# azrael417/mlperf-deepcam

Hardware: AMD Instinct MI355X
Metric: samples/sec (768x1152x16) train step (higher is better)
Workload: dtype bf16; 1 GPU; DeepLabV3+/Xception train step (fwd + weighted CE + bwd + LAMB), 768x1152x16, local_batch=8, bf16 activations / fp32 master weights, random-init seed 333; local_batch=8, global_batch=8, parallelism=dp1, optimizer=LAMB, hip_graph=False, launch_list_replay=False

## Files before the change

mlperf-deepcam_amd/csrc/common.h:

```cpp
#pragma once
#include <hip/hip_runtime.h>
#include <stdint.h>

#include <mutex>

#include "../../include/deepcam_hip.h"

namespace dc {

typedef __bf16 bf16;
typedef __attribute__((ext_vector_type(8))) __bf16 bf16x8;
typedef __attribute__((ext_vector_type(4))) __bf16 bf16x4;
typedef __attribute__((ext_vector_type(4))) short short4v;
typedef __attribute__((ext_vector_type(4))) float f32x4;
typedef __attribute__((ext_vector_type(2))) float f32x2;

struct alignas(16) vec16 {
  uint32_t w[4];
};

template <typename T>
struct Elem;
template <>
struct Elem<float> {
  static constexpr int kPerVec = 4;
  static constexpr int kDtype = DC_F32;
  __device__ static inline float load(const float* p) { return *p; }
  __device__ static inline void store(float* p, float v) { *p = v; }
};
template <>
struct Elem<bf16> {
  static constexpr int kPerVec = 8;
  static constexpr int kDtype = DC_BF16;
  __device__ static inline float load(const bf16* p) { return (float)*p; }
  __device__ static inline void store(bf16* p, float v) { *p = (bf16)v; }
};

__device__ inline void unpack(const vec16& v, float (&f)[4], float) {
#pragma unroll
  for (int i = 0; i < 4; ++i) f[i] = __uint_as_float(v.w[i]);
}
__device__ inline void unpack(const vec16& v, float (&f)[8], bf16) {
#pragma unroll
  for (int i = 0; i < 4; ++i) {
    f[2 * i] = __uint_as_float(v.w[i] << 16);
    f[2 * i + 1] = __uint_as_float(v.w[i] & 0xffff0000u);
  }
}
__device__ inline uint32_t pack2_bf16(float lo, float hi) {
  typedef __attribute__((ext_vector_type(2))) __bf16 bf16x2;
  bf16x2 r;
  r[0] = (bf16)lo;
  r[1] = (bf16)hi;
  return __builtin_bit_cast(uint32_t, r);
}
__device__ inline void pack(vec16& v, const float (&f)[4], float) {
#pragma unroll
  for (int i = 0; i < 4; ++i) v.w[i] = __float_as_uint(f[i]);
}
__device__ inline void pack(vec16& v, const float (&f)[8], bf16) {
#pragma unroll
  for (int i = 0; i < 4; ++i) v.w[i] = pack2_bf16(f[2 * i], f[2 * i + 1]);
}

__device__ inline vec16 zero16() {
  vec16 z;
  z.w[0] = z.w[1] = z.w[2] = z.w[3] = 0u;
  return z;
}
__device__ inline vec16 ldg16(const void* p) { return *reinterpret_cast<const vec16*>(p); }
__device__ inline void stg16(void* p, const vec16& v) { *reinterpret_cast<vec16*>(p) = v; }

__device__ inline float wave_sum(float v) {
#pragma unroll
  for (int o = 32; o > 0; o >>= 1) v += __shfl_xor(v, o, 64);
  return v;
}
__device__ inline double wave_sum(double v) {
#pragma unroll
  for (int o = 32; o > 0; o >>= 1) v += __shfl_xor(v, o, 64);
  return v;
}

inline int cdiv(long a, long b) { return (int)((a + b - 1) / b); }

struct Options {
  int igemm256 = 1;
  int igemm256p = 1;
  int igemm256p_wgs = 0;
  int igemm256p_min = 257;
  int igemm256_splitk = 1;
  int pw384 = 1;
  int pw224 = 1;
  int pw192 = 1;
  int thin_tile = 1;
  int wgrad384 = 1;
  int wgrad384_slots = 192;
  int wgrad384_min_stages = 96;
  int head_fused = 1;
  int head_dgrad_fused = 1;
  int head_wgrad_fused = 1;
  int dw_tile = 1;
  int dw_wgrad_tpb = 0;
  int dw_pipe = 1;
  int bn_apply_rows = 1;
};
extern Options g_options;

const void* zero_page(hipError_t* err);

}

#define DC_ONCE(...)                               \
  do {                                             \
    static std::once_flag once_flag__;             \
    std::call_once(once_flag__, [&] { __VA_ARGS__; }); \
  } while (0)

namespace dc {
extern thread_local bool g_launch_log_on;
void launch_log_note(const char* name);
}

#define DC_LAUNCHED(name)                                  \
  do {                                                     \
    hipError_t e__ = hipGetLastError();                    \
    if (e__ != hipSuccess) return dc_set_error(e__, __FILE__, __LINE__); \
    if (dc::g_launch_log_on) dc::launch_log_note(name);    \
  } while (0)
#define DC_CHECK_LAUNCH() DC_LAUNCHED("aux")

extern "C" int dc_set_error(int code, const char* file, int line);
extern "C" int dc_fail(const char* msg, const char* file, int line);
extern "C" int dc_check_view(const void* ptr, int ld, int c, int dtype, const char* what);
#define DC_REQUIRE(cond, msg)                                  \
  do {                                                         \
    if (!(cond)) return dc_fail(msg, __FILE__, __LINE__);      \
  } while (0)
```

mlperf-deepcam_amd/csrc/igemm.h:

```cpp
#pragma once
#include "conv_geom.h"

namespace dc {

constexpr int WLD_ALIGN = 64;
__host__ __device__ inline int weight_ld(int c) {
  const int a = c < 64 ? 32 : WLD_ALIGN;
  return (c + a - 1) / a * a;
}


struct BnBwdEpi {
  const void* y;
  int ldy;
  const float* mean;
  const float* invstd;
  const float* mscale;
  const float* mshift;
  int relu;
};

struct IgemmParams {
  const void* x;
  const void* w;
  void* y;
  const float* bias;
  float* slab;
  GatherGeom g;
  int N, ldx, ldy;
  int ldw;
  const void* w_kn = nullptr;
  int ldw_kn = 0;
  int M;
  int m_beg = 0;
  int mtiles;
  int accumulate = 0;
  const void* zero_page = nullptr;
  static constexpr int MAXGROUP = 4;
  BnBwdEpi bst{};
  int ngroup = 0;
  int gdil[MAXGROUP];
  const void* gw[MAXGROUP - 1];
  void* gy[MAXGROUP - 1];
  float* gslab[MAXGROUP - 1];
  int ksplit = 0;
  float* kslab = nullptr;
  int zfill = 0;
};

int launch_igemm256(const IgemmParams& p, hipStream_t st);
bool igemm256p_eligible(const IgemmParams& p);
int launch_igemm256p(const IgemmParams& p, int workgroups, hipStream_t st);
inline long igemm256_tiles(const IgemmParams& p) {
  return (long)((p.g.Cout + 255) / 256) * ((p.M - p.m_beg + 255) / 256) * p.g.os * p.g.os * (p.ngroup > 1 ? p.ngroup : 1);
}
int igemm256_splitk_plan(const IgemmParams& p, size_t* slab_bytes);
int launch_igemm256_splitk(const IgemmParams& p, int splits, void* ws, hipStream_t st);

bool pw384_eligible(const IgemmParams& p);
int launch_pw384(const IgemmParams& p, int npb, hipStream_t st);
inline long pw384_tiles(const IgemmParams& p, int npb) { return (long)((p.g.Cout + 383) / 384) * ((p.M + 32 * npb - 1) / (32 * npb)); }

bool pw224_eligible(const IgemmParams& p);
int launch_pw224(const IgemmParams& p, int tn, hipStream_t st);
inline long pw224_tiles(const IgemmParams& p, int tn = 384) { return (long)((p.g.Cout + tn - 1) / tn) * ((p.M + 223) / 224); }

long pw192_tiles(const IgemmParams& p);
int launch_pw192(const IgemmParams& p, hipStream_t st);

bool thin_fwd_eligible(const GatherGeom& g, int dtype, int bias, int accumulate, int out32);
int launch_thin_fwd(const GatherGeom& g, int N, const void* in, int ldin, const void* w, int ldw, void* out, int ldout, float* slab,
                    int slab_rows, hipStream_t st);

}
```

mlperf-deepcam_amd/csrc/igemm.hip:

```cpp
#include <stdio.h>
#include <string.h>

#include <type_traits>

#include "conv_geom.h"
#include "igemm.h"
#include "mfma_tile.h"

namespace dc {

constexpr int BM = 128, BN = 128;
constexpr int ROWB = 64, NSTAGE = 3;

template <typename T>
struct Mma;
template <>
struct Mma<bf16> {
  __device__ static inline void run(const vec16& a, const vec16& b, f32x4& c) {
    c = __builtin_amdgcn_mfma_f32_16x16x32_bf16(__builtin_bit_cast(bf16x8, a), __builtin_bit_cast(bf16x8, b), c, 0, 0, 0);
  }
};
template <>
struct Mma<float> {
  __device__ static inline void run(const vec16& a, const vec16& b, f32x4& c) {
// ... 665 lines not shown
    int lo = 0, hi = nentries;
    while (hi - lo > 1) {
      const int mid = (lo + hi) >> 1;
      if (prefix[mid] <= gt) lo = mid; else hi = mid;
    }
    const PackEntry e = table[lo];
    const int tile = gt - prefix[lo];
    if (e.kind == 2) {
      float* out = reinterpret_cast<float*>(e.wf);
      const int c = tile * 256 + threadIdx.x;
      if (c < e.cout) {
#pragma unroll
        for (int t = 0; t < 9; ++t) out[(size_t)t * e.cout + c] = e.master[(size_t)c * 9 + t];
      }
      continue;
    }
    if (e.taps == 1) {
      if constexpr (sizeof(T) == 2) {
        if (((e.cin | e.cout) & 7) == 0) pack_pointwise_tile_bf16(e, tile, lds);
        else pack_dense_tile<T, 1>(e, tile, lds);
      } else {
        pack_dense_tile<T, 1>(e, tile, lds);
      }
    } else {
      pack_dense_tile<T, 9>(e, tile, lds);
    }
  }
}

}

using namespace dc;

constexpr int PACK_BLOCKS = 2048;
extern "C" int dc_pack_all(int dtype, const void* table_dev, int nentries, void* stream) {
  DC_REQUIRE(table_dev != nullptr && nentries > 0, "dc_pack_all: bad argument");
  DC_REQUIRE(sizeof(PackEntry) == 40, "dc_pack_all: entry layout changed");
  DC_REQUIRE(nentries <= PACK_MAX_ENTRIES, "dc_pack_all: too many entries for one launch");
  dim3 grid(PACK_BLOCKS);
  if (dtype == DC_BF16) hipLaunchKernelGGL(pack_all_kernel<bf16>, grid, dim3(256), 0, (hipStream_t)stream, (const PackEntry*)table_dev, nentries);
  else hipLaunchKernelGGL(pack_all_kernel<float>, grid, dim3(256), 0, (hipStream_t)stream, (const PackEntry*)table_dev, nentries);
  DC_CHECK_LAUNCH();
  return 0;
}

Options dc::g_options;

static __device__ __attribute__((aligned(256))) unsigned char dc_arg_zero_page[256];

const void* dc::zero_page(hipError_t* err) {
  static void* dev = nullptr;
  static hipError_t init_err = hipSuccess;
  DC_ONCE({ init_err = hipGetSymbolAddress(&dev, HIP_SYMBOL(dc_arg_zero_page)); });
  *err = init_err;
  return dev;
}

namespace {
enum class Norm { kValue, kFlag, kZeroToTwo, kNonNegative, kPositive, kStages };
const struct {
  const char* name;
  int Options::*field;
  Norm norm;
} kOptions[] = {
    {"igemm256", &Options::igemm256, Norm::kValue},
    {"igemm256p", &Options::igemm256p, Norm::kValue},
    {"igemm256p_wgs", &Options::igemm256p_wgs, Norm::kValue},
    {"igemm256p_min", &Options::igemm256p_min, Norm::kValue},
    {"igemm256_splitk", &Options::igemm256_splitk, Norm::kValue},
    {"pw384", &Options::pw384, Norm::kValue},
    {"pw224", &Options::pw224, Norm::kValue},
    {"pw192", &Options::pw192, Norm::kValue},
    {"thin_tile", &Options::thin_tile, Norm::kFlag},
    {"wgrad384", &Options::wgrad384, Norm::kValue},
    {"wgrad384_slots", &Options::wgrad384_slots, Norm::kPositive},
    {"wgrad384_min_stages", &Options::wgrad384_min_stages, Norm::kStages},
    {"head_fused", &Options::head_fused, Norm::kFlag},
    {"head_dgrad_fused", &Options::head_dgrad_fused, Norm::kFlag},
    {"head_wgrad_fused", &Options::head_wgrad_fused, Norm::kFlag},
    {"dw_tile", &Options::dw_tile, Norm::kFlag},
    {"dw_wgrad_tpb", &Options::dw_wgrad_tpb, Norm::kNonNegative},
    {"dw_pipe", &Options::dw_pipe, Norm::kZeroToTwo},
    {"bn_apply_rows", &Options::bn_apply_rows, Norm::kFlag},
};
}

extern "C" int dc_set_option(const char* name, int value) {
  for (const auto& o : kOptions) {
    if (name == nullptr || strcmp(name, o.name) != 0) continue;
    switch (o.norm) {
      case Norm::kValue: break;
      case Norm::kFlag: value = value != 0; break;
      case Norm::kZeroToTwo: value = value < 0 ? 0 : value > 2 ? 2 : value; break;
      case Norm::kNonNegative: value = value < 0 ? 0 : value; break;
      case Norm::kPositive:
      case Norm::kStages:
        if (value < 1) {
          char msg[96];
          snprintf(msg, sizeof(msg), "dc_set_option: %s must be positive", o.name);
          return dc_fail(msg, __FILE__, __LINE__);
        }
        if (o.norm == Norm::kStages && value < 4) value = 4;
        break;
    }
    g_options.*o.field = value;
    return 0;
  }
  return dc_fail("dc_set_option: unknown option", __FILE__, __LINE__);
}

extern "C" int dc_reset_options(void) {
  g_options = Options{};
  return 0;
}

extern "C" int dc_conv_out_hw(const dc_conv_desc* d, int Hi, int Wi, int* Ho, int* Wo) {
  DC_REQUIRE(d != nullptr, "dc_conv_out_hw: null descriptor");
  GatherGeom g;
  if (!build_geom(*d, Hi, Wi, kFwd, &g)) return dc_fail("dc_conv_out_hw: unsupported geometry", __FILE__, __LINE__);
  if (Ho) *Ho = g.Hout;
  if (Wo) *Wo = g.Wout;
  return 0;
}

extern "C" int dc_conv_stat_rows(const dc_conv_desc* d, int N, int Hi, int Wi) {
  GatherGeom g;
  if (d == nullptr || !build_geom(*d, Hi, Wi, kFwd, &g)) return -1;
  return cdiv((long)N * g.Qh * g.Qw, BM) * g.os * g.os;
}

extern "C" int dc_conv_fwd(const dc_conv_desc* d, int N, int Hi, int Wi, const void* x, int ldx, const void* wf,
                           const float* bias, void* y, int ldy, float* stat_slab, int accumulate, void* stream) {
  return run_gather(d, kFwd, N, Hi, Wi, x, ldx, wf, bias, y, ldy, stat_slab, accumulate, stream);
}

extern "C" int dc_conv_fwd_kn(const dc_conv_desc* d, int N, int Hi, int Wi, const void* x, int ldx, const void* wf, const void* wb,
                              const float* bias, void* y, int ldy, float* stat_slab, int slab_rows, int accumulate, void* stream) {
  return run_gather(d, kFwd, N, Hi, Wi, x, ldx, wf, bias, y, ldy, stat_slab, accumulate, stream, false, nullptr, wb, slab_rows);
}
static int kn_forward_plan(const dc_conv_desc* d, int N, int Hi, int Wi, long* Mout) {
  const int plain = dc_conv_stat_rows(d, N, Hi, Wi);
  if (plain <= 0 || d->dtype != DC_BF16) return 0;
  IgemmParams p;
  if (!build_geom(*d, Hi, Wi, kFwd, &p.g)) return 0;
  const long M = (long)N * p.g.Qh * p.g.Qw;
  if (M >= (1L << 31) - BM) return 0;
  if (M <= TINY_M || thin_fwd_eligible(p.g, d->dtype, false, 0, false)) return 0;
  p.x = nullptr; p.w = nullptr; p.y = nullptr; p.bias = nullptr; p.slab = nullptr;
  p.N = N; p.ldx = weight_ld(p.g.Cin); p.ldy = weight_ld(p.g.Cout); p.ldw = weight_ld(p.g.Cin);
  alignas(16) static const char some_image[16] = {0};
  p.w_kn = some_image;
  p.ldw_kn = weight_ld(p.g.Cout);
  p.M = (int)M;
  p.mtiles = cdiv(M, BM);
  *Mout = M;
  return pw384_plan(p);
}
extern "C" int dc_conv_stat_rows_kn(const dc_conv_desc* d, int N, int Hi, int Wi) {
  long M = 0;
  const int npb = kn_forward_plan(d, N, Hi, Wi, &M);
  return (npb == 224 || npb == 226) ? cdiv(M, 224) : dc_conv_stat_rows(d, N, Hi, Wi);
}
extern "C" int dc_conv_sum_row_kn(const dc_conv_desc* d, int N, int Hi, int Wi) {
  if (d == nullptr) return 0;
  long M = 0;
  const int npb = kn_forward_plan(d, N, Hi, Wi, &M);
// ... 130 lines not shown
```

mlperf-deepcam_amd/csrc/igemm256.hip:

```cpp
#include <type_traits>

#include "igemm.h"
#include "mfma_tile.h"

namespace dc {

namespace {

constexpr int TM = 256, TN = 256;
constexpr int ROWB = 64;
constexpr int BK = 32;
constexpr int NSTAGE = 4;
constexpr int OPER = TM * ROWB;
constexpr int STAGE = 2 * OPER;
constexpr int RING = NSTAGE * STAGE;
constexpr int CROW = TN * 2 + 16;
constexpr int CTILE = TM * CROW;
constexpr int MAIN_BYTES = RING > CTILE ? RING : CTILE;

__global__ __launch_bounds__(512) void igemm256_kernel(const IgemmParams p) {
  extern __shared__ __attribute__((aligned(16))) char smem[];
  int* s_tap = reinterpret_cast<int*>(smem + MAIN_BYTES);
  const GatherGeom& g = p.g;
  const int tid = threadIdx.x, lane = tid & 63;
  const int wave = __builtin_amdgcn_readfirstlane(tid >> 6);
  const int grp = wave >> 2;
  const int wc = wave & 3;

  const int ntn = (g.Cout + TN - 1) / TN;
  const int nwg = gridDim.x;
  const int q8 = nwg >> 3, r8 = nwg & 7, xcd = blockIdx.x & 7, xslot = blockIdx.x >> 3;
  int tile = (xcd < r8 ? xcd * (q8 + 1) : r8 * (q8 + 1) + (xcd - r8) * q8) + xslot;
  const int nsplit = p.ksplit > 1 ? p.ksplit : 1;
  const int tiles_per_split = nwg / nsplit;
  const int split = tile / tiles_per_split;
  tile -= split * tiles_per_split;
  const int tile_lin = tile;
  const int ntile_n = tile % ntn;
  int rest = tile / ntn;
  const int ngroup = p.ngroup > 1 ? p.ngroup : 1;
  const int member = rest % ngroup;
  rest /= ngroup;
  const void* wsel = p.w;
  void* ysel = p.y;
  float* slabsel = p.slab;
  int dilmul = p.ngroup > 1 ? p.gdil[0] : 1;
#pragma unroll
  for (int b = 1; b < IgemmParams::MAXGROUP; ++b)
    if (member == b) {
      wsel = p.gw[b - 1];
      ysel = p.gy[b - 1];
      slabsel = p.gslab[b - 1];
      dilmul = p.gdil[b];
    }
  const int nph = g.os * g.os;
  const int phase = rest % nph;
  const int mtile = rest / nph;
  const int n0 = ntile_n * TN, m0 = p.m_beg + mtile * TM;
  const int py = phase / g.os, px = phase % g.os;

  const int tap_beg = g.phase_beg[phase], ntap = g.phase_beg[phase + 1] - tap_beg;
  if (tid < ntap) {
    const Tap tp = g.taps[tap_beg + tid];
    s_tap[3 * tid] = tp.dy * dilmul;
    s_tap[3 * tid + 1] = tp.dx * dilmul;
    s_tap[3 * tid + 2] = tp.widx;
  }
  __syncthreads();
  const int kchunks_all = (g.Cin + BK - 1) / BK;
  constexpr int KG = 4;
  const int ngk = (kchunks_all + KG - 1) / KG;
  const int kfirst = nsplit > 1 ? (ngk * split / nsplit) * KG : 0;
  const int kchunks = nsplit > 1 ? min(kchunks_all, (ngk * (split + 1) / nsplit) * KG) : kchunks_all;
  const int steps = ntap * (kchunks - kfirst);
  if (steps == 0 && p.accumulate) return;

  const int lrow = lane >> 2, pslot = lane & 3;
  const int lslot = pslot ^ ((lrow >> 1) & 3);
  const bf16* __restrict__ xg = reinterpret_cast<const bf16*>(p.x);
  const bf16* __restrict__ wg = reinterpret_cast<const bf16*>(wsel);
  int rown[2], riy[2], rix[2];
  bool rok[2];
#pragma unroll
  for (int j = 0; j < 2; ++j) {
    const int m = m0 + (8 * j + wave) * 16 + lrow;
    rok[j] = m < p.M;
    const int mm = rok[j] ? m : 0;
    int n, qy, qx;
    grid_pixel(g, mm, n, qy, qx);
    rown[j] = n * g.Hin;
    riy[j] = qy * g.is;
    rix[j] = qx * g.is;
  }
  const bf16* xrow[2] = {xg, xg};
  const bf16* wrow[2] = {wg, wg};
  bool xok[2] = {false, false}, wok[2] = {false, false};
  int tapA = -1, tapB = -1;
  const uintptr_t zp = (uintptr_t)p.zero_page;
  auto pick = [&](bool ok, const bf16* a) { return (gas_ptr)(ok ? (uintptr_t)a : zp); };
  auto issue_A = [&](int tapi, int kc, int slot, bool live) {
    if (live && tapi != tapA) {
      tapA = tapi;
      const int widx = s_tap[3 * tapi + 2];
#pragma unroll
      for (int j = 0; j < 2; ++j) {
        const int ch = n0 + (8 * j + wave) * 16 + lrow;
        wok[j] = ch < g.Cout;
        wrow[j] = wg + (((size_t)widx * g.Cout + (wok[j] ? ch : 0)) * p.ldw + lslot * 8);
      }
    }
    const int kofs = kc * BK;
    const bool kok = live & (kofs + lslot * 8 < g.Cin);
    char* base = smem + slot * STAGE;
#pragma unroll
    for (int j = 0; j < 2; ++j)
      __builtin_amdgcn_global_load_lds(pick(kok & wok[j], wrow[j] + kofs), (lds_ptr)(base + (8 * j + wave) * 16 * ROWB), 16, 0, 0);
  };
  auto issue_B = [&](int tapi, int kc, int slot, bool live) {
    if (live && tapi != tapB) {
      tapB = tapi;
      const int dy = s_tap[3 * tapi], dx = s_tap[3 * tapi + 1];
#pragma unroll
      for (int j = 0; j < 2; ++j) {
        const int iy = riy[j] + dy, ix = rix[j] + dx;
        xok[j] = rok[j] && (unsigned)iy < (unsigned)g.Hin && (unsigned)ix < (unsigned)g.Win;
        xrow[j] = xg + (((size_t)(rown[j] + (xok[j] ? iy : 0)) * g.Win + (xok[j] ? ix : 0)) * p.ldx + lslot * 8);
      }
    }
    const int kofs = kc * BK;
    const bool kok = live & (kofs + lslot * 8 < g.Cin);
    char* base = smem + slot * STAGE + OPER;
#pragma unroll
    for (int j = 0; j < 2; ++j)
      __builtin_amdgcn_global_load_lds(pick(kok & xok[j], xrow[j] + kofs), (lds_ptr)(base + (8 * j + wave) * 16 * ROWB), 16, 0, 0);
  };

  f32x4 acc[4][8];
#pragma unroll
  for (int i = 0; i < 4; ++i)
#pragma unroll
    for (int j = 0; j < 8; ++j) acc[i][j] = f32x4{0.f, 0.f, 0.f, 0.f};
  const int fr = lane & 15, fg = lane >> 4;

  int itap = 0, ikc = kfirst;
  int kbeg = kfirst, kend = kchunks < kfirst + KG ? kchunks : kfirst + KG;
  auto advance = [&]() {
    if (++ikc == kend) {
      ikc = kbeg;
      if (++itap == ntap) {
        itap = 0;
        kbeg = kend;
// ... 246 lines not shown
  __shared__ float red[2][4][TN];
  const int half = blockIdx.x & 1;
  const int tile_lin = blockIdx.x >> 1;
  const int ntile_n = tile_lin % a.ntn;
  int rest = tile_lin / a.ntn;
  const int member = rest % a.ngroup;
  const int mtile = rest / a.ngroup;
  bf16* yg = nullptr;
  float* sl = nullptr;
#pragma unroll
  for (int b = 0; b < IgemmParams::MAXGROUP; ++b)
    if (member == b) {
      yg = reinterpret_cast<bf16*>(a.y[b]);
      sl = a.slab[b];
    }
  const int cg = threadIdx.x & 63, rl = threadIdx.x >> 6;
  const int ch = ntile_n * TN + cg * 4;
  const bool chok = ch < a.Cout;
  const size_t tstride = (size_t)a.tiles_per_split * (TM * TN);
  const float* base = a.kslab + (size_t)tile_lin * (TM * TN) + (size_t)(half * 128) * TN + cg * 4;
  float ssum[4] = {0.f, 0.f, 0.f, 0.f}, ssq[4] = {0.f, 0.f, 0.f, 0.f};
  for (int r = rl; r < 128; r += 4) {
    const int m = mtile * TM + half * 128 + r;
    if (m >= a.M || !chok) continue;
    f32x4 v = *reinterpret_cast<const f32x4*>(base + (size_t)r * TN);
    for (int s = 1; s < a.nsplit; ++s) v += *reinterpret_cast<const f32x4*>(base + s * tstride + (size_t)r * TN);
    uint2 o;
    o.x = pack2_bf16(v[0], v[1]);
    o.y = pack2_bf16(v[2], v[3]);
    *reinterpret_cast<uint2*>(yg + (size_t)m * a.ldy + ch) = o;
    if (sl != nullptr) {
      const float f[4] = {__uint_as_float(o.x << 16), __uint_as_float(o.x & 0xffff0000u), __uint_as_float(o.y << 16), __uint_as_float(o.y & 0xffff0000u)};
#pragma unroll
      for (int e = 0; e < 4; ++e) {
        ssum[e] += f[e];
        ssq[e] = fmaf(f[e], f[e], ssq[e]);
      }
    }
  }
  if (sl == nullptr) return;
#pragma unroll
  for (int e = 0; e < 4; ++e) {
    red[0][rl][cg * 4 + e] = ssum[e];
    red[1][rl][cg * 4 + e] = ssq[e];
  }
  __syncthreads();
  const int mt128 = mtile * 2 + half;
  for (int i = threadIdx.x; i < 2 * TN; i += 256) {
    const int c = i % TN, which = i / TN;
    if (ntile_n * TN + c < a.Cout && mt128 < a.mtiles)
      sl[((size_t)which * a.mtiles + mt128) * a.Cout + ntile_n * TN + c] = (red[which][0][c] + red[which][1][c]) + (red[which][2][c] + red[which][3][c]);
  }
}

int igemm256_splitk_plan(const IgemmParams& p, size_t* slab_bytes) {
  if (slab_bytes) *slab_bytes = 0;
  if (!g_options.igemm256_splitk || p.g.os != 1 || p.m_beg != 0 || p.bias != nullptr || p.accumulate || p.bst.y != nullptr || (p.g.Cout & 7)) return 1;
  const long tiles = igemm256_tiles(p);
  if (tiles < 1) return 1;
  const int ngk = ((p.g.Cin + BK - 1) / BK + 3) / 4;
  int s = 1;
  if (tiles <= 128) {
    s = (int)(256 / tiles);
    if (s > ngk / 2) s = ngk / 2;
    if (s > 8) s = 8;
  } else if (g_options.igemm256_splitk > 1) {
    auto fill = [](long n) { return (double)n / (double)(((n + 255) / 256) * 256); };
    double best = fill(tiles) + 0.10;
    for (int c = 2; c <= 4 && c <= ngk / 2; ++c)
      if (fill(tiles * c) > best) {
        best = fill(tiles * c);
        s = c;
      }
  }
  if (s < 2) return 1;
  if (slab_bytes) *slab_bytes = (size_t)s * tiles * TM * TN * sizeof(float);
  return s;
}

int launch_igemm256(const IgemmParams& p_in, hipStream_t st) {
  const size_t lds = (size_t)MAIN_BYTES + 128;
  DC_ONCE({ (void)hipFuncSetAttribute(reinterpret_cast<const void*>(&igemm256_kernel), hipFuncAttributeMaxDynamicSharedMemorySize, (int)lds); });
  IgemmParams p = p_in;
  hipError_t zerr;
  p.zero_page = zero_page(&zerr);
  if (zerr != hipSuccess) return dc_set_error(zerr, __FILE__, __LINE__);
  hipLaunchKernelGGL(igemm256_kernel, dim3((unsigned)(igemm256_tiles(p) * (p.ksplit > 1 ? p.ksplit : 1))), dim3(512), lds, st, p);
  DC_LAUNCHED(p.ksplit > 1 ? "igemm256_splitk" : "igemm256");
  return 0;
}

int launch_igemm256_splitk(const IgemmParams& p_in, int splits, void* ws, hipStream_t st) {
  IgemmParams p = p_in;
  p.ksplit = splits;
  p.kslab = reinterpret_cast<float*>(ws);
  if (int e = launch_igemm256(p, st)) return e;
  SplitKFoldArgs a;
  a.kslab = p.kslab; a.nsplit = splits; a.tiles_per_split = (int)igemm256_tiles(p); a.ntn = (p.g.Cout + TN - 1) / TN;
  a.ngroup = p.ngroup > 1 ? p.ngroup : 1; a.mt256 = (p.M + TM - 1) / TM; a.mtiles = p.mtiles; a.M = p.M; a.Cout = p.g.Cout; a.ldy = p.ldy;
  for (int b = 0; b < IgemmParams::MAXGROUP; ++b) {
    a.y[b] = b == 0 ? p.y : p.gy[b - 1];
    a.slab[b] = b == 0 ? p.slab : p.gslab[b - 1];
  }
  hipLaunchKernelGGL(igemm256_splitk_fold_kernel, dim3((unsigned)(2 * a.tiles_per_split)), dim3(256), 0, st, a);
  DC_LAUNCHED("igemm256_splitk_fold");
  return 0;
}

}
```

mlperf-deepcam_amd/csrc/wgrad384.hip:

```cpp
#include "mfma_tile.h"
#include "wgrad.h"

namespace dc {

namespace {

constexpr int TCO = 256, TCI = 384;
constexpr int BP = 32;
constexpr int QUAD = BP * 128;
constexpr int QT = (TCO / 64) * QUAD;
constexpr int PT = (TCI / 64) * QUAD;
constexpr int STAGE = QT + PT;
constexpr int NI = STAGE / 1024;
constexpr int IPW = NI / 8;
constexpr int NCB = 12;
constexpr int NPB = 4;
constexpr int LATE = NCB - 1 - IPW;
constexpr int NST = 4;
constexpr int DMA_AUX = 0;
static_assert(NI % 8 == 0 && NST * STAGE <= 160 * 1024 && NST >= 3, "ring");

typedef __attribute__((ext_vector_type(2))) uint32_t u32x2;
typedef __attribute__((ext_vector_type(4))) uint32_t u32x4;

struct Wg384Params {
  const void* zero_page;
  int Cin, Cout, ldx, lddy;
  int M, splits, chunk, nlayers;
  int ntaps, cq, H, W;
  int tdy[9], tdx[9], twidx[9];
  FastDiv div_hw, div_w;
  const void* x[WG384_MAXL];
  const void* dy[WG384_MAXL];
  float* out[WG384_MAXL];
};

template <int OFF>
__device__ inline void lds_read_frag(bf16x8& dst, uint32_t addr) {
  static_assert(OFF >= 0 && OFF + 16 * 128 < 65536, "ds_read offset field");
  u32x2 lo, hi;
  asm volatile("ds_read_b64_tr_b16 %0, %1 offset:%2" : "=v"(lo) : "v"(addr), "n"(OFF) : "memory");
  asm volatile("ds_read_b64_tr_b16 %0, %1 offset:%2" : "=v"(hi) : "v"(addr), "n"(OFF + 16 * 128) : "memory");
  u32x4 f;
  f[0] = lo[0]; f[1] = lo[1]; f[2] = hi[0]; f[3] = hi[1];
  dst = __builtin_bit_cast(bf16x8, f);
}
template <typename T>
__device__ inline T karg(size_t field_offset, int index) {
  const char* ka = (const char*)__builtin_amdgcn_kernarg_segment_ptr();
  return *(const T*)(ka + field_offset + sizeof(T) * index);
}

template <int MODE>
__global__ __launch_bounds__(512) void wgrad384_kernel(const Wg384Params p) {
  constexpr bool TAPS = MODE != 0;
  extern __shared__ __attribute__((aligned(16))) char smem[];
  const int tid = threadIdx.x, lane = tid & 63;
  const int wave = __builtin_amdgcn_readfirstlane(tid >> 6);
  const int grp = wave >> 1;
  const int wc = wave & 1;
  const bool late = wave >= 4;

  const int nq = p.ntaps * p.cq;
  const int nxt = (nq + 5) / 6, nco = (p.Cout + TCO - 1) / TCO;
  const int nwg = gridDim.x;
  const int q8 = nwg >> 3, r8 = nwg & 7, xcd = blockIdx.x & 7, xslot = blockIdx.x >> 3;
  int tile = (xcd < r8 ? xcd * (q8 + 1) : r8 * (q8 + 1) + (xcd - r8) * q8) + xslot;
  const int q0 = (tile % nxt) * 6;
  tile /= nxt;
  const int co0 = (tile % nco) * TCO;
  tile /= nco;
  const int split = tile % p.splits, layer = tile / p.splits;
  const int mbeg = split * p.chunk;
  const int mend = min(p.M, mbeg + p.chunk);
  const int npix = mend > mbeg ? mend - mbeg : 0;
  const int steps = (npix + BP - 1) / BP;
  const uintptr_t xbase = karg<uintptr_t>(__builtin_offsetof(Wg384Params, x), layer);
  const uintptr_t dbase = karg<uintptr_t>(__builtin_offsetof(Wg384Params, dy), layer);
  float* const obase = karg<float*>(__builtin_offsetof(Wg384Params, out), layer);
  const uintptr_t zp = (uintptr_t)p.zero_page;

  const int drow = 8 * (wave & 3) + (lane >> 3);
  const int dsub = ((lane & 7) >> 1) ^ ((drow >> 1) & 3);
  const int dch = dsub * 16 + (lane & 1) * 8;
  const unsigned lsrc_d = (unsigned)((drow * p.lddy + dch) * 2);
  typename std::conditional<MODE == 2, long, unsigned>::type lsrc_x = (unsigned)((drow * p.ldx + dch) * 2);
  const int gw = MODE == 2 ? 2 * p.W : p.W, gh = MODE == 2 ? 2 * p.H : p.H;
  int dlim[2], xlim[3], tdy[3], tdx[3];
  long doff[2], xoff[3];
#pragma unroll
  for (int i = 0; i < 2; ++i) {
    const int c = co0 + (2 * i + (wave >> 2)) * 64;
    doff[i] = (long)c * 2;
    dlim[i] = p.Cout - c;
  }
#pragma unroll
  for (int k = 0; k < 3; ++k) {
    const int q = q0 + 2 * k + (wave >> 2);
    const int tap = q / p.cq, ciq = q - tap * p.cq;
    const bool qok = q < nq;
    const int tt = qok ? tap : 0;
    tdy[k] = TAPS ? karg<int>(__builtin_offsetof(Wg384Params, tdy), tt) : 0;
    tdx[k] = TAPS ? karg<int>(__builtin_offsetof(Wg384Params, tdx), tt) : 0;
    xoff[k] = ((long)(tdy[k] * gw + tdx[k]) * p.ldx + ciq * 64) * 2;
    xlim[k] = qok ? p.Cin - ciq * 64 : 0;
  }
  const size_t dstep = (size_t)BP * p.lddy * 2, xstep = (size_t)(MODE == 2 ? 4 * BP : BP) * p.ldx * 2;
  uintptr_t dcur = dbase + (size_t)mbeg * p.lddy * 2, xcur = xbase + (size_t)(MODE == 2 ? 4 : 1) * mbeg * p.ldx * 2;
  int rows_left = npix;
  int oy = 0, ox = 0;
  if constexpr (TAPS) {
    const int m = mbeg + drow < p.M ? mbeg + drow : 0;
    const int n = fast_div(m, p.div_hw);
    const int rem = m - n * (p.H * p.W);
    oy = fast_div(rem, p.div_w);
    ox = rem - oy * p.W;
    if constexpr (MODE == 2) lsrc_x = ((long)(4 * drow - 2 * ox) * p.ldx + dch) * 2;
  }
  auto issue = [&](int i, int slot) {
    bool ok = drow < rows_left;
    uintptr_t a;
    if (i < 2) {
      ok &= dch < dlim[i];
      a = dcur + doff[i] + lsrc_d;
    } else {
      const int k = i - 2;
      ok &= dch < xlim[k];
      if constexpr (MODE == 1) ok &= ((unsigned)(oy + tdy[k]) < (unsigned)gh) & ((unsigned)(ox + tdx[k]) < (unsigned)gw);
      if constexpr (MODE == 2) ok &= ((unsigned)(2 * oy + tdy[k]) < (unsigned)gh) & ((unsigned)(2 * ox + tdx[k]) < (unsigned)gw);
      a = xcur + xoff[k] + lsrc_x;
    }
    __builtin_amdgcn_global_load_lds((gas_ptr)(ok ? a : zp), (lds_ptr)(smem + slot * STAGE + (8 * i + wave) * 1024), 16, 0, DMA_AUX);
  };
  auto advance = [&]() {
    dcur += dstep;
    xcur += xstep;
    rows_left -= BP;
    if constexpr (TAPS) {
      ox += BP;
      if (ox >= p.W) {
        ox -= p.W;
        oy = oy + 1 == p.H ? 0 : oy + 1;
      }
      if constexpr (MODE == 2) lsrc_x = ((long)(4 * drow - 2 * ox) * p.ldx + dch) * 2;
    }
  };

  constexpr int LATE_PRIO = 1;
  if (late) __builtin_amdgcn_s_setprio(LATE_PRIO);
  f32x4 acc[NCB][NPB];
#pragma unroll
  for (int i = 0; i < NCB; ++i)
#pragma unroll
    for (int j = 0; j < NPB; ++j) acc[i][j] = f32x4{0.f, 0.f, 0.f, 0.f};

  const int fr = lane & 15, fg = lane >> 4;
  const int frow = 4 * fg + (fr >> 2);
  const int fkey = (frow >> 1) & 3;
  const uint32_t lds0 = (uint32_t)(uintptr_t)(lds_ptr)smem;
  uint32_t la[4], lb[4];
#pragma unroll
  for (int s = 0; s < 4; ++s) {
    const uint32_t l = (uint32_t)(frow * 128 + ((s ^ fkey) << 5) + 8 * (fr & 3));
    la[s] = lds0 + QT + wc * 3 * QUAD + l;
    lb[s] = lds0 + grp * QUAD + l;
  }
  static_assert(NCB % 3 == 0, "fa ring");
  bf16x8 fa[3], fb[NPB];

  auto step = [&](uint32_t cur, uint32_t nxt, int dslot) {
    static_for<0, NCB>([&](auto ic) {
      constexpr int i = decltype(ic)::value;
      if constexpr (i + 2 < NCB) lds_read_frag<((i + 2) >> 2) * QUAD>(fa[(i + 2) % 3], la[(i + 2) & 3] + cur);
      if constexpr (i < IPW) {
        if (!late) issue(i, dslot);
      }
      if constexpr (i >= LATE && i < LATE + IPW) {
        if (late) issue(i - LATE, dslot);
      }
      if constexpr (i == NCB - 1) {
        asm volatile("s_waitcnt vmcnt(%0) lgkmcnt(0)" ::"n"((NST - 2) * IPW) : "memory");
        __builtin_amdgcn_s_barrier();
        lds_read_frag<0>(fa[0], la[0] + nxt);
        lds_read_frag<0>(fa[1], la[1] + nxt);
      }
      static_for<0, NPB>([&](auto jc) {
        constexpr int j = decltype(jc)::value;
        if constexpr (i == 0) lgkm_wait<2 * (NPB - j)>();
        else if constexpr (j == 0 && i < NCB - 1) lgkm_wait<2 * (NCB - 1 - i < 2 ? NCB - 1 - i : 2)>();
        mfma_v(acc[i][j], fa[i % 3], fb[j]);
        if constexpr (i == NCB - 1) lds_read_frag<0>(fb[j], lb[j] + nxt);
      });
    });
  };

#pragma unroll
  for (int q = 0; q < NST - 1; ++q) {
#pragma unroll
    for (int i = 0; i < IPW; ++i) issue(i, q);
    advance();
  }
  asm volatile("s_waitcnt vmcnt(%0)" ::"n"((NST - 2) * IPW) : "memory");
  __builtin_amdgcn_s_barrier();
  lds_read_frag<0>(fa[0], la[0]);
  lds_read_frag<0>(fa[1], la[1]);
  static_for<0, NPB>([&](auto jc) { lds_read_frag<0>(fb[decltype(jc)::value], lb[decltype(jc)::value]); });
  int cslot = 0;
  for (int s = 0; s < steps; ++s) {
    const int nslot = cslot + 1 == NST ? 0 : cslot + 1;
    const int dslot = cslot == 0 ? NST - 1 : cslot - 1;
    step((uint32_t)(cslot * STAGE), (uint32_t)(nslot * STAGE), dslot);
    advance();
    cslot = nslot;
  }
  asm volatile("s_waitcnt vmcnt(0) lgkmcnt(0)\n\ts_nop 15\n\ts_nop 15" ::: "memory");

#pragma unroll
  for (int k = 0; k < 3; ++k) {
    const int q = q0 + wc * 3 + k;
    if (q >= nq) continue;
    const int tap = q / p.cq, ciq = q - tap * p.cq;
    const int plane = split * p.ntaps + (TAPS ? karg<int>(__builtin_offsetof(Wg384Params, twidx), tap) : 0);
    if constexpr (MODE != 2) {
      float* out = obase + (size_t)plane * p.Cout * p.Cin + ciq * 64;
#pragma unroll
      for (int j = 0; j < NPB; ++j) {
        const int co = co0 + grp * 64 + j * 16 + fr;
        if (co >= p.Cout) continue;
        float* orow = out + (size_t)co * p.Cin;
#pragma unroll
        for (int ii = 0; ii < 4; ++ii) {
          const int c = ii * 16 + fg * 4;
          if (ciq * 64 + c < p.Cin) *reinterpret_cast<f32x4*>(orow + c) = acc[4 * k + ii][j];
        }
      }
    } else {
      float* out = obase + (size_t)plane * p.Cout * p.Cin;
#pragma unroll
      for (int j = 0; j < NPB; ++j) {
        const int cx = co0 + grp * 64 + j * 16 + fr;
        if (cx >= p.Cout) continue;
#pragma unroll
        for (int ii = 0; ii < 4; ++ii) {
          const int cg = ciq * 64 + ii * 16 + fg * 4;
          if (cg >= p.Cin) continue;
#pragma unroll
          for (int r = 0; r < 4; ++r) out[(size_t)(cg + r) * p.Cout + cx] = acc[4 * k + ii][j][r];
        }
      }
    }
  }
}

}

bool wgrad384_is_tconv(const GatherGeom& g) {
  return g.os == 2 && g.is == 1 && g.ntaps == 9 && g.Hout == 2 * g.Hin && g.Wout == 2 * g.Win;
}

bool wgrad384_eligible(const GatherGeom& g, int ldx, int lddy, long M) {
  if (g.Cin % 8 != 0 || g.Cout % 8 != 0) return false;
  if (wgrad384_is_tconv(g)) return g.Win >= BP && (size_t)4 * BP * (ldx > lddy ? ldx : lddy) * 2 + 4096 < (1ull << 31);
  if (g.os != 1 || g.is != 1 || g.ntaps < 1 || g.ntaps > 9) return false;
  if ((size_t)BP * ldx * 2 + 2 * TCI >= (1ull << 32) || (size_t)BP * lddy * 2 + 2 * TCO >= (1ull << 32)) return false;
  if (g.ntaps == 1) return g.taps[0].dy == 0 && g.taps[0].dx == 0;
  if (g.Hin != g.Hout || g.Win != g.Wout || g.Win < BP) return false;
  for (int t = 0; t < g.ntaps; ++t)
    if (g.taps[t].phase != 0 || g.taps[t].dy <= -g.Hin || g.taps[t].dy >= g.Hin || g.taps[t].dx <= -g.Win || g.taps[t].dx >= g.Win) return false;
  (void)M;
  return true;
}

static long wgrad384_tiles(const GatherGeom& g) {
  if (wgrad384_is_tconv(g)) return (long)cdiv((long)g.ntaps * cdiv(g.Cout, 64), 6) * cdiv(g.Cin, TCO);
  return (long)cdiv((long)g.ntaps * cdiv(g.Cin, 64), 6) * cdiv(g.Cout, TCO);
}
void wgrad384_plan(const GatherGeom& g, long M, int* splits, int* chunk, int group) {
  const long tiles = wgrad384_tiles(g) * group;
  long want = g_options.wgrad384_slots / tiles;
  const long per = (long)g_options.wgrad384_min_stages * BP;
  const long maxs = (M + per - 1) / per;
  if (want > maxs) want = maxs;
  if (want < 1) want = 1;
  long c = (M + want - 1) / want;
  c = (c + BP - 1) / BP * BP;
  *chunk = (int)c;
  *splits = (int)((M + c - 1) / c);
}

int launch_wgrad384(const WgradParams& w, hipStream_t st, int group, const void* const* xs, const void* const* dys, float* const* outs) {
  const size_t lds = (size_t)NST * STAGE;
  DC_ONCE({
    (void)hipFuncSetAttribute(reinterpret_cast<const void*>(&wgrad384_kernel<0>), hipFuncAttributeMaxDynamicSharedMemorySize, (int)lds);
    (void)hipFuncSetAttribute(reinterpret_cast<const void*>(&wgrad384_kernel<1>), hipFuncAttributeMaxDynamicSharedMemorySize, (int)lds);
    (void)hipFuncSetAttribute(reinterpret_cast<const void*>(&wgrad384_kernel<2>), hipFuncAttributeMaxDynamicSharedMemorySize, (int)lds);
  });
  hipError_t zerr;
  const void* zero_dev = zero_page(&zerr);
  if (zerr != hipSuccess) return dc_set_error(zerr, __FILE__, __LINE__);
  if (group < 1 || group > WG384_MAXL) return dc_fail("launch_wgrad384: group size out of range", __FILE__, __LINE__);
  const GatherGeom& g = w.g;
  if (!wgrad384_eligible(g, w.ldx, w.lddy, w.M) || w.ldx < g.Cin || w.lddy < g.Cout)
    return dc_fail("launch_wgrad384: geometry or row strides outside what the kernel serves", __FILE__, __LINE__);
  Wg384Params pp;
  pp.zero_page = zero_dev;
  pp.Cin = g.Cin; pp.Cout = g.Cout; pp.ldx = w.ldx; pp.lddy = w.lddy;
  pp.M = w.M; pp.splits = w.splits; pp.chunk = w.chunk; pp.nlayers = group;
  pp.ntaps = g.ntaps; pp.cq = cdiv(g.Cin, 64); pp.H = g.Hin; pp.W = g.Win;
  for (int t = 0; t < 9; ++t) {
    pp.tdy[t] = t < g.ntaps ? g.taps[t].dy : 0;
    pp.tdx[t] = t < g.ntaps ? g.taps[t].dx : 0;
    pp.twidx[t] = t < g.ntaps ? g.taps[t].widx : 0;
  }
  pp.div_hw = g.div_hw; pp.div_w = g.div_w;
  for (int l = 0; l < WG384_MAXL; ++l) {
    pp.x[l] = l < group ? (group == 1 && xs == nullptr ? w.x : xs[l]) : nullptr;
    pp.dy[l] = l < group ? (group == 1 && dys == nullptr ? w.dy : dys[l]) : nullptr;
    pp.out[l] = l < group ? (group == 1 && outs == nullptr ? w.slab : outs[l]) : nullptr;
  }
  const long blocks = wgrad384_tiles(g) * w.splits * group;
  if (wgrad384_is_tconv(g)) {
    pp.Cin = g.Cout; pp.Cout = g.Cin; pp.ldx = w.lddy; pp.lddy = w.ldx;
    pp.cq = cdiv(g.Cout, 64); pp.H = g.Hin; pp.W = g.Win;
    for (int t = 0; t < 9; ++t) {
      const int widx = t < g.ntaps ? g.taps[t].widx : 0;
      pp.tdy[t] = widx / 3 - 1;
      pp.tdx[t] = widx % 3 - 1;
    }
    pp.div_hw = make_fastdiv(g.Hin * g.Win);
    pp.div_w = make_fastdiv(g.Win);
    for (int l = 0; l < WG384_MAXL; ++l) {
      const void* t = pp.x[l];
      pp.x[l] = pp.dy[l];
      pp.dy[l] = t;
    }
    hipLaunchKernelGGL(wgrad384_kernel<2>, dim3((unsigned)blocks), dim3(512), lds, st, pp);
  } else if (g.ntaps == 1) hipLaunchKernelGGL(wgrad384_kernel<0>, dim3((unsigned)blocks), dim3(512), lds, st, pp);
  else hipLaunchKernelGGL(wgrad384_kernel<1>, dim3((unsigned)blocks), dim3(512), lds, st, pp);
  DC_LAUNCHED(wgrad384_is_tconv(g) ? "wgrad384_convT" : g.ntaps == 1 ? "wgrad384_pw" : "wgrad384_3x3");
  return 0;
}

}
```

Before: 264.6 samples/s.

## Skip convolution taps and pixel blocks that fall entirely in padding

```diff
diff --git a/mlperf-deepcam_amd/csrc/common.h b/mlperf-deepcam_amd/csrc/common.h
--- a/mlperf-deepcam_amd/csrc/common.h
+++ b/mlperf-deepcam_amd/csrc/common.h
@@ -104,6 +104,7 @@
   int dw_wgrad_tpb = 0;
   int dw_pipe = 1;
   int bn_apply_rows = 1;
+  int skip_empty_taps = 1;
 };
 extern Options g_options;
 
diff --git a/mlperf-deepcam_amd/csrc/igemm.h b/mlperf-deepcam_amd/csrc/igemm.h
--- a/mlperf-deepcam_amd/csrc/igemm.h
+++ b/mlperf-deepcam_amd/csrc/igemm.h
@@ -45,6 +45,7 @@
   float* gslab[MAXGROUP - 1];
   int ksplit = 0;
   float* kslab = nullptr;
+  int skip_empty_taps = 0;
   int zfill = 0;
 };
 
diff --git a/mlperf-deepcam_amd/csrc/igemm.hip b/mlperf-deepcam_amd/csrc/igemm.hip
--- a/mlperf-deepcam_amd/csrc/igemm.hip
+++ b/mlperf-deepcam_amd/csrc/igemm.hip
@@ -771,6 +771,7 @@
     {"dw_wgrad_tpb", &Options::dw_wgrad_tpb, Norm::kNonNegative},
     {"dw_pipe", &Options::dw_pipe, Norm::kZeroToTwo},
     {"bn_apply_rows", &Options::bn_apply_rows, Norm::kFlag},
+    {"skip_empty_taps", &Options::skip_empty_taps, Norm::kFlag},
 };
 }
 
diff --git a/mlperf-deepcam_amd/csrc/igemm256.hip b/mlperf-deepcam_amd/csrc/igemm256.hip
--- a/mlperf-deepcam_amd/csrc/igemm256.hip
+++ b/mlperf-deepcam_amd/csrc/igemm256.hip
@@ -59,14 +59,38 @@
   const int n0 = ntile_n * TN, m0 = p.m_beg + mtile * TM;
   const int py = phase / g.os, px = phase % g.os;
 
-  const int tap_beg = g.phase_beg[phase], ntap = g.phase_beg[phase + 1] - tap_beg;
-  if (tid < ntap) {
-    const Tap tp = g.taps[tap_beg + tid];
-    s_tap[3 * tid] = tp.dy * dilmul;
-    s_tap[3 * tid + 1] = tp.dx * dilmul;
-    s_tap[3 * tid + 2] = tp.widx;
+  const int tap_beg = g.phase_beg[phase], ntap_all = g.phase_beg[phase + 1] - tap_beg;
+  if (wave == 0) {
+    bool alive = false;
+    int tdy = 0, tdx = 0, twidx = 0;
+    if (tid < ntap_all) {
+      const Tap tp = g.taps[tap_beg + tid];
+      tdy = tp.dy * dilmul;
+      tdx = tp.dx * dilmul;
+      twidx = tp.widx;
+      alive = !p.skip_empty_taps || ntap_all == 1;
+      const int m1 = min(p.M, m0 + TM);
+      const int qx_lo = tdx < 0 ? (-tdx + g.is - 1) / g.is : 0;
+      for (int m = m0; m < m1 && !alive;) {
+        int n, qy, qx;
+        grid_pixel(g, m, n, qy, qx);
+        const int len = min(m1 - m, g.Qw - qx);
+        const int qxa = max(qx, qx_lo);
+        alive = (unsigned)(qy * g.is + tdy) < (unsigned)g.Hin && qxa < qx + len && qxa * g.is + tdx < g.Win;
+        m += len;
+      }
+    }
+    const unsigned long long live = __ballot(alive);
+    if (alive) {
+      const int pos = __popcll(live & ((1ull << tid) - 1ull));
+      s_tap[3 * pos] = tdy;
+      s_tap[3 * pos + 1] = tdx;
+      s_tap[3 * pos + 2] = twidx;
+    }
+    if (tid == 0) s_tap[27] = __popcll(live);
   }
   __syncthreads();
+  const int ntap = __builtin_amdgcn_readfirstlane(s_tap[27]);
   const int kchunks_all = (g.Cin + BK - 1) / BK;
   constexpr int KG = 4;
   const int ngk = (kchunks_all + KG - 1) / KG;
@@ -479,6 +503,7 @@
   const size_t lds = (size_t)MAIN_BYTES + 128;
   DC_ONCE({ (void)hipFuncSetAttribute(reinterpret_cast<const void*>(&igemm256_kernel), hipFuncAttributeMaxDynamicSharedMemorySize, (int)lds); });
   IgemmParams p = p_in;
+  p.skip_empty_taps = g_options.skip_empty_taps;
   hipError_t zerr;
   p.zero_page = zero_page(&zerr);
   if (zerr != hipSuccess) return dc_set_error(zerr, __FILE__, __LINE__);
diff --git a/mlperf-deepcam_amd/csrc/wgrad384.hip b/mlperf-deepcam_amd/csrc/wgrad384.hip
--- a/mlperf-deepcam_amd/csrc/wgrad384.hip
+++ b/mlperf-deepcam_amd/csrc/wgrad384.hip
@@ -28,6 +28,7 @@
   int Cin, Cout, ldx, lddy;
   int M, splits, chunk, nlayers;
   int ntaps, cq, H, W;
+  int skip_empty;
   int tdy[9], tdx[9], twidx[9];
   FastDiv div_hw, div_w;
   const void* x[WG384_MAXL];
@@ -74,7 +75,7 @@
   const int mbeg = split * p.chunk;
   const int mend = min(p.M, mbeg + p.chunk);
   const int npix = mend > mbeg ? mend - mbeg : 0;
-  const int steps = (npix + BP - 1) / BP;
+  int steps = (npix + BP - 1) / BP;
   const uintptr_t xbase = karg<uintptr_t>(__builtin_offsetof(Wg384Params, x), layer);
   const uintptr_t dbase = karg<uintptr_t>(__builtin_offsetof(Wg384Params, dy), layer);
   float* const obase = karg<float*>(__builtin_offsetof(Wg384Params, out), layer);
@@ -109,6 +110,34 @@
   uintptr_t dcur = dbase + (size_t)mbeg * p.lddy * 2, xcur = xbase + (size_t)(MODE == 2 ? 4 : 1) * mbeg * p.ldx * 2;
   int rows_left = npix;
   int oy = 0, ox = 0;
+  [[maybe_unused]] int dead_a = 0, dead_b = 0, srem = 0, sy = 0, sx = 0;
+  if constexpr (MODE == 1) {
+    const int hw = p.H * p.W;
+    srem = mbeg - fast_div(mbeg < p.M ? mbeg : 0, p.div_hw) * hw;
+    sy = fast_div(srem, p.div_w);
+    sx = srem - sy * p.W;
+    if (p.skip_empty && steps > 0) {
+      int hi = -1, lo = p.H;
+      for (int k = 0; k < 6; ++k) {
+        const int q = q0 + k < nq ? q0 + k : nq - 1;
+        const int dy = karg<int>(__builtin_offsetof(Wg384Params, tdy), q / p.cq);
+        if (dy >= 0) hi = max(hi, p.H - 1 - dy);
+        if (dy <= 0) lo = min(lo, -dy);
+      }
+      if (hi + 1 < lo) {
+        dead_a = (hi + 1) * p.W;
+        dead_b = lo * p.W;
+        const int j0 = mbeg / BP, j1 = j0 + steps;
+        const int nlast = fast_div(mend - 1, p.div_hw);
+        int empty = 0;
+        for (int n = fast_div(mbeg, p.div_hw); n <= nlast; ++n) {
+          const int ja = max(j0, (n * hw + dead_a + BP - 1) / BP), jb = min(j1, (n * hw + dead_b) / BP);
+          if (jb > ja) empty += jb - ja;
+        }
+        steps -= empty;
+      }
+    }
+  }
   if constexpr (TAPS) {
     const int m = mbeg + drow < p.M ? mbeg + drow : 0;
     const int n = fast_div(m, p.div_hw);
@@ -122,21 +151,58 @@
     uintptr_t a;
     if (i < 2) {
       ok &= dch < dlim[i];
-      a = dcur + doff[i] + lsrc_d;
+      if constexpr (MODE == 1) {
+        uintptr_t sb = dcur + doff[i];
+        asm volatile("" : "+s"(sb));
+        a = sb + lsrc_d;
+      } else {
+        a = dcur + doff[i] + lsrc_d;
+      }
     } else {
       const int k = i - 2;
       ok &= dch < xlim[k];
       if constexpr (MODE == 1) ok &= ((unsigned)(oy + tdy[k]) < (unsigned)gh) & ((unsigned)(ox + tdx[k]) < (unsigned)gw);
       if constexpr (MODE == 2) ok &= ((unsigned)(2 * oy + tdy[k]) < (unsigned)gh) & ((unsigned)(2 * ox + tdx[k]) < (unsigned)gw);
-      a = xcur + xoff[k] + lsrc_x;
+      if constexpr (MODE == 1) {
+        uintptr_t sb = xcur + xoff[k];
+        asm volatile("" : "+s"(sb));
+        a = sb + lsrc_x;
+      } else {
+        a = xcur + xoff[k] + lsrc_x;
+      }
     }
     __builtin_amdgcn_global_load_lds((gas_ptr)(ok ? a : zp), (lds_ptr)(smem + slot * STAGE + (8 * i + wave) * 1024), 16, 0, DMA_AUX);
+  };
+  [[maybe_unused]] auto seek_live = [&]() {
+    while (rows_left > 0 && srem >= dead_a && srem + BP <= dead_b) {
+      const int run = min((dead_b - srem) / BP, (rows_left + BP - 1) / BP);
+      dcur += (size_t)run * dstep;
+      xcur += (size_t)run * xstep;
+      rows_left -= run * BP;
+      srem += run * BP;
+      if (srem >= p.H * p.W) srem -= p.H * p.W;
+      sy = fast_div(srem, p.div_w);
+      sx = srem - sy * p.W;
+    }
+    const int sy1 = sy + 1 == p.H ? 0 : sy + 1;
+    const bool wrap = sx + drow >= p.W;
+    ox = sx + drow - (wrap ? p.W : 0);
+    oy = wrap ? sy1 : sy;
   };
   auto advance = [&]() {
     dcur += dstep;
     xcur += xstep;
     rows_left -= BP;
-    if constexpr (TAPS) {
+    if constexpr (MODE == 1) {
+      srem += BP;
+      if (srem >= p.H * p.W) srem -= p.H * p.W;
+      sx += BP;
+      if (sx >= p.W) {
+        sx -= p.W;
+        sy = sy + 1 == p.H ? 0 : sy + 1;
+      }
+      seek_live();
+    } else if constexpr (TAPS) {
       ox += BP;
       if (ox >= p.W) {
         ox -= p.W;
@@ -194,6 +260,7 @@
     });
   };
 
+  if constexpr (MODE == 1) seek_live();
 #pragma unroll
   for (int q = 0; q < NST - 1; ++q) {
 #pragma unroll
@@ -266,7 +333,7 @@
   if (g.ntaps == 1) return g.taps[0].dy == 0 && g.taps[0].dx == 0;
   if (g.Hin != g.Hout || g.Win != g.Wout || g.Win < BP) return false;
   for (int t = 0; t < g.ntaps; ++t)
-    if (g.taps[t].phase != 0 || g.taps[t].dy <= -g.Hin || g.taps[t].dy >= g.Hin || g.taps[t].dx <= -g.Win || g.taps[t].dx >= g.Win) return false;
+    if (g.taps[t].phase != 0 || g.taps[t].dx <= -g.Win || g.taps[t].dx >= g.Win) return false;
   (void)M;
   return true;
 }
@@ -307,6 +374,7 @@
   pp.Cin = g.Cin; pp.Cout = g.Cout; pp.ldx = w.ldx; pp.lddy = w.lddy;
   pp.M = w.M; pp.splits = w.splits; pp.chunk = w.chunk; pp.nlayers = group;
   pp.ntaps = g.ntaps; pp.cq = cdiv(g.Cin, 64); pp.H = g.Hin; pp.W = g.Win;
+  pp.skip_empty = g_options.skip_empty_taps;
   for (int t = 0; t < 9; ++t) {
     pp.tdy[t] = t < g.ntaps ? g.taps[t].dy : 0;
     pp.tdx[t] = t < g.ntaps ? g.taps[t].dx : 0;
```

New measurement: 265.3 samples/s, median of 6. About the same (+0.3%).
